# MatteoSoldini/metamorphic_testing_of_the_MUSICA_Algorithm_for_x_ray_image_processing

Hardware: AMD Instinct MI355X
Metric: megapixels/sec full MUSICA pipeline (higher is better)
Workload: dtype f32

## Files before the change

devtools/random_parity.py:

```python
import os
import sys

ROOT = os.path.dirname(os.path.dirname(os.path.abspath(__file__)))
sys.path.insert(0, ROOT)
sys.path.insert(0, os.path.join(ROOT, "tests"))
import numpy as np
from metamorphic_testing_of_the_musica_algorithm_for_x_ray_image_processing_amd import processing as mp
from metamorphic_testing_of_the_musica_algorithm_for_x_ray_image_processing_amd.phantom import phantom
from oracle import binding as ob
import test_gpu_parity as tp

cases = int(sys.argv[1]) if len(sys.argv) > 1 else 30
rng = np.random.default_rng(int(sys.argv[2]) if len(sys.argv) > 2 else 7)
ob.set_threads(min(16, os.cpu_count() or 1))
knobs = ["MUSICA_SDEV_IN_EXPAND", "MUSICA_PAIR_RB_SDEV", "MUSICA_SDEV_ONE_LAUNCH", "MUSICA_GRAPH", "MUSICA_AUTOTUNE", "MUSICA_TINY_TAIL"]
for case in range(cases):
    n = int(rng.choice([8 * int(rng.integers(8, 190)), int(rng.integers(64, 1500))]))
    lmax = int(np.ceil(np.log2(n)))
    levels = int(rng.integers(4, lmax + 1))
    batch = int(rng.choice([1, 1, 2, 3]))
    clahe = bool(rng.integers(0, 4) == 0) and n >= 64
    linear = bool(rng.integers(0, 2))
    env = {k: str(int(rng.integers(0, 2))) for k in knobs}
    env["MUSICA_STREAMS"] = str(int(rng.integers(1, 3)))
    for k, v in env.items():
        os.environ[k] = v
    flags = (mp.FLAG_CLAHE if clahe else 0) | (mp.FLAG_LINEAR if linear else 0)
    px = np.stack([phantom(n, 5000 + 10 * case + k) for k in range(batch)])
    p = mp.MusicaProcessing()
    assert p.init(n, levels=levels, batch=batch, flags=flags), mp.last_error()
# ... 9 lines not shown
```

include/musica.h:

```cpp
#ifndef MUSICA_H
#define MUSICA_H

#include <stddef.h>
#include <stdint.h>

#ifdef __cplusplus
extern "C" {
#endif

#define MUSICA_ABI_VERSION 3

#define MUSICA_MAX_LEVELS 16
#define MUSICA_MIN_LEVELS 4
#define MUSICA_NOISE_BINS 2048
#define MUSICA_GRAD_BINS 1024
#define MUSICA_MAX_POINTS 256
#define MUSICA_CNR_LEVEL 3
#define MUSICA_COARSER_LEVELS_START 3
#define MUSICA_OUT_MARGIN 10
#define MUSICA_CLAHE_TILES 4
#define MUSICA_CLAHE_BINS 256

typedef struct musica_hist_max_point {
    uint32_t maxValue;
// ... 100 lines not shown

musica_ctx* musica_create(const musica_params* params);
musica_ctx* musica_create_ex(const musica_params* params, const musica_tunables* tunables);
void musica_tunables_default(musica_tunables* out);
int musica_get_tunables(const musica_ctx* ctx, musica_tunables* out);

void musica_destroy(musica_ctx* ctx);

uint32_t musica_get_image_size(const musica_ctx* ctx);
uint32_t musica_get_levels(const musica_ctx* ctx);
uint32_t musica_get_batch(const musica_ctx* ctx);
int musica_fuses_gradation_histogram(const musica_ctx* ctx);
int musica_fuses_reduce_band(const musica_ctx* ctx);
int musica_fuses_sdev(const musica_ctx* ctx);
int musica_get_paired_levels(const musica_ctx* ctx);
uint32_t musica_get_level_size(const musica_ctx* ctx, uint32_t level);
int musica_get_dispatch(const musica_ctx* ctx, int* streams, int* graph);


int musica_execute(musica_ctx* ctx, const uint16_t* pixels);

int musica_execute_device(musica_ctx* ctx, const uint16_t* d_pixels);

int musica_upload(musica_ctx* ctx, const uint16_t* pixels);
const uint16_t* musica_input_device_ptr(musica_ctx* ctx);

int musica_sync(musica_ctx* ctx);


int musica_get_graded(musica_ctx* ctx, float* dst);
// ... 233 lines not shown
```

metamorphic_testing_of_the_musica_algorithm_for_x_ray_image_processing_amd/csrc/kernels_pyramid.hip:

```cpp
#include <stdlib.h>
#include <type_traits>
#include "kernels_common.h"
#include "sdev_parts.h"
#include "launchers.h"

#ifndef MUSICA_PYRAMID_SD_ONLY
#define MUSICA_PYRAMID_FULL 1
#endif

namespace musica {

struct LaneCfg {
    int c;
    bool active;
    bool left_mirror;
    bool last_active;
    bool lane0, lane63;
    uint32_t off;
    uint32_t off_l;
    uint32_t off_r;
    uint32_t coff;
    uint32_t coff_l;
    uint32_t coff_r;
};
// ... 324 lines not shown
}
template <class R>
__device__ __forceinline__ void band_pair(const CRow& a, const CRow& b, const CRow& c, const R& fe, const R& fo, const LaneCfg& g,
                                          const Buf& bb, uint32_t off_e, uint32_t off_o) {
    float lowE[8], lowO[8], be[8], bo[8];
    lowpass_pair(a, b, c, g, lowE, lowO);
#pragma unroll
    for (int j = 0; j < 8; j++) {
        be[j] = fe.v[j] - lowE[j];
        bo[j] = fo.v[j] - lowO[j];
    }
    store8_nt(bb, g.off + off_e, be);
    store8_nt(bb, g.off + off_o, bo);
}

__device__ __forceinline__ uint32_t le090_bits(const FRowQ& fe, const FRowQ& fo) {
    uint32_t m = 0u;
#pragma unroll
    for (int j = 0; j < 8; j++) {
        m |= fe.v[j] <= 0.90f ? 1u << j : 0u;
        m |= fo.v[j] <= 0.90f ? 1u << (8 + j) : 0u;
    }
    return m;
}

__device__ __forceinline__ void load_f(FRow& r, const Buf& b, uint32_t row_off, uint32_t off, uint32_t off_h) {
    load8(r.v, b, off + row_off);
    const float4 h = bload4(b, off_h + row_off);
    r.h[0] = h.x; r.h[1] = h.y; r.h[2] = h.z; r.h[3] = h.w;
}

template <bool U16>
__device__ __forceinline__ void reduce_band_block(const void* __restrict__ fine, float* __restrict__ down, float* __restrict__ band,
                                                  int S, int pitch, size_t plane, int Sc, int cpitch, size_t cplane,
                                                  int rows_per_wave, const uint32_t* __restrict__ minmax, int min_chain_exact,
                                                  uint16_t* __restrict__ le090, const Tile tile, const int img) {
    const int lane = threadIdx.x & 63;
    const int seg = __builtin_amdgcn_readfirstlane((int)(tile.segblock * kWavesPerBlock + (threadIdx.x >> 6)));
    const int k0 = seg * rows_per_wave;
    if (k0 >= Sc) return;
    const int k1 = min(k0 + rows_per_wave, Sc);
    NormK nk = make_norm(0.0f, 1.0f);
    if (U16) {
        float minv, maxv;
        chain_scalars(minmax, img, min_chain_exact, minv, maxv);
        nk = make_norm(minv, maxv);
    }
    const Buf ib = U16 ? make_buf(reinterpret_cast<const uint16_t*>(fine) + (size_t)img * S * S, (size_t)S * S * 2)
                       : make_buf(reinterpret_cast<const float*>(fine) + (size_t)img * plane, plane * 4);
    const Buf db = make_buf(down + (size_t)img * cplane, cplane * 4);
    const Buf bb = make_buf(band + (size_t)img * plane, plane * 4);
    const LaneCfg g = make_cfg(tile.strip, lane, S);
    const bool want_mask = U16 && le090 != nullptr;
    const Buf mb = want_mask ? make_buf(le090 + (size_t)img * Sc * (S / 8), (size_t)Sc * (S / 8) * 2) : bb;
    const uint32_t moff = g.off == kOob ? kOob : (uint32_t)g.c >> 2, mrb = (uint32_t)S >> 2;
    const uint32_t px_bytes = U16 ? 2u : 4u;
    const uint32_t foff = g.off == kOob ? kOob : (uint32_t)g.c * px_bytes;
    const uint32_t foff_h = g.off_l != kOob ? (uint32_t)(g.c - 4) * px_bytes : (g.off_r != kOob ? (uint32_t)(g.c + 8) * px_bytes : kOob);
    const uint32_t qi = (uint32_t)lane & 3u;
    const int hi = S - 1;
    const uint32_t frb = U16 ? (uint32_t)S * 2u : (uint32_t)pitch * 4u, rb = (uint32_t)pitch * 4u, crb = (uint32_t)cpitch * 4u;
    const int ks = max(k0 - 1, 0), ke = min(k1, Sc - 1);

    typename std::conditional<U16, FRowQ, FRow>::type w0, w1, w2, w3, w4;
    RawF ra, rc;
    if constexpr (U16) {
        load_raw_f(ra, ib, (uint32_t)mirror_idx(2 * ks - 2, hi) * frb, foff, foff_h);
        convert_f(w0, ra, nk, qi);
        load_raw_f(ra, ib, (uint32_t)mirror_idx(2 * ks - 1, hi) * frb, foff, foff_h);
        convert_f(w1, ra, nk, qi);
        load_raw_f(ra, ib, (uint32_t)(2 * ks) * frb, foff, foff_h);
        convert_f(w2, ra, nk, qi);
        load_raw_f(ra, ib, (uint32_t)mirror_idx(2 * ks + 1, hi) * frb, foff, foff_h);
        load_raw_f(rc, ib, (uint32_t)mirror_idx(2 * ks + 2, hi) * frb, foff, foff_h);
    } else {
        load_f(w0, ib, (uint32_t)mirror_idx(2 * ks - 2, hi) * frb, foff, foff_h);
        load_f(w1, ib, (uint32_t)mirror_idx(2 * ks - 1, hi) * frb, foff, foff_h);
        load_f(w2, ib, (uint32_t)(2 * ks) * frb, foff, foff_h);
    }
    CRow c0, cm1, cm2;
    cm1 = CRow(); cm2 = CRow();
    for (int k = ks; k <= ke; k++) {
        if constexpr (U16) {
            convert_f(w3, ra, nk, qi);
            convert_f(w4, rc, nk, qi);
            const int kn = min(k + 1, ke);
            load_raw_f(ra, ib, (uint32_t)mirror_idx(2 * kn + 1, hi) * frb, foff, foff_h);
            load_raw_f(rc, ib, (uint32_t)mirror_idx(2 * kn + 2, hi) * frb, foff, foff_h);
        } else {
            load_f(w3, ib, (uint32_t)mirror_idx(2 * k + 1, hi) * frb, foff, foff_h);
            load_f(w4, ib, (uint32_t)mirror_idx(2 * k + 2, hi) * frb, foff, foff_h);
        }
        coarse_row(c0, w0, w1, w2, w3, w4, g);
        if (k >= k0 && k < k1)
            bstore4_nt(db, g.coff + (uint32_t)k * crb, make_float4(c0.v[0], c0.v[1], c0.v[2], c0.v[3]));
        const int kp = k - 1;
        if (kp >= k0 && kp < k1) {
            if constexpr (U16) if (want_mask) bstore_u16(mb, moff + (uint32_t)kp * mrb, le090_bits(w0, w1));
            band_pair(kp == 0 ? c0 : cm2, cm1, c0, w0, w1, g, bb, (uint32_t)(2 * kp) * rb, (uint32_t)(2 * kp + 1) * rb);
        }
        cm2 = cm1; cm1 = c0;
        w0 = w2; w1 = w3; w2 = w4;
    }
    if (k1 == Sc) {
        if constexpr (U16) if (want_mask) bstore_u16(mb, moff + (uint32_t)(Sc - 1) * mrb, le090_bits(w0, w1));
        band_pair(cm2, cm1, cm1, w0, w1, g, bb, (uint32_t)(2 * (Sc - 1)) * rb, (uint32_t)(2 * (Sc - 1) + 1) * rb);
    }
}
template <bool U16>
__global__ __launch_bounds__(kBlockThreads, 4) void k_reduce_band(const void* __restrict__ fine, float* __restrict__ down, float* __restrict__ band,
                                                               int S, int pitch, size_t plane, int Sc, int cpitch, size_t cplane,
                                                               int rows_per_wave, const uint32_t* __restrict__ minmax, int min_chain_exact,
                                                               uint16_t* __restrict__ le090, int swz) {
    reduce_band_block<U16>(fine, down, band, S, pitch, plane, Sc, cpitch, cplane, rows_per_wave, minmax, min_chain_exact, le090, xcd_tile(swz), (int)blockIdx.z);
}

__device__ __forceinline__ float lowpass_generic(const float* __restrict__ coarse, int cpitch, int Sc, int S, int x, int y, int ref) {
    if (ref) {
        float pixel = 0.0f;
#pragma unroll
        for (int m = 0; m < 5; m++) {
// ... 526 lines not shown
    return dim3(strips, (segs + kWavesPerBlock - 1) / kWavesPerBlock, batch);
}

#ifndef MUSICA_PYRAMID_FULL
__device__ __forceinline__ bool role_tile(int local, int strips, int blocks, int swz, Tile& t) {
    if (swz && (blocks & 7) == 0) {
        const int xcd = local & 7, j = local >> 3;
        t.strip = j % strips;
        t.segblock = xcd * (blocks >> 3) + j / strips;
    } else {
        t.strip = local % strips;
        t.segblock = local / strips;
    }
    return t.segblock < blocks;
}
__global__ __launch_bounds__(kBlockThreads, 4) void k_rb_sdev(const RbSdevArgs a) {
    __shared__ uint32_t lh[kHistLdsWords];
    __shared__ unsigned long long nzw[kWavesPerBlock][8];
    const int img = (int)blockIdx.z;
    Tile tile;
    if ((int)blockIdx.x >= a.rb_first) {
        if (!role_tile((int)blockIdx.x - a.rb_first, a.rb_strips, a.rb_blocks, a.swz, tile)) return;
        reduce_band_block<false>(a.fine, a.down, a.band, a.S, a.pitch, a.plane, a.Sc, a.cpitch, a.cplane, a.rows_rb, nullptr, 0, nullptr, tile, img);
        return;
    }
    const SdevRunLevel& l = a.sl;
    if (!role_tile((int)blockIdx.x, l.strips, l.blocks, a.swz, tile)) return;
    float* sd = l.sdev ? l.sdev + (size_t)img * l.plane : nullptr;
    if (l.rows > 0) sdev_march_block<true, true>(l.band + (size_t)img * l.plane, sd, l.S, l.pitch, l.plane, l.hist + (size_t)img * a.hist_stride, a.cov, l.rows, tile, lh);
    else sdev_run_block<true>(l.band + (size_t)img * l.plane, sd, l.S, l.pitch, l.plane, l.hist + (size_t)img * a.hist_stride, a.cov, tile, lh, nzw);
}
void launch_rb_sdev(hipStream_t st, RbSdevArgs a, const LevelDesc& ls, int batch) {
    const int s_strips = (ls.S + kStripCols - 1) / kStripCols;
    int s_blocks;
    if (a.sl.rows > 0) { const int segs = (ls.S + a.sl.rows - 1) / a.sl.rows; s_blocks = (segs + kWavesPerBlock - 1) / kWavesPerBlock; }
    else s_blocks = (ls.S + kHistArea - 1) / kHistArea;
    a.sl.plane = ls.plane; a.sl.S = ls.S; a.sl.pitch = ls.pitch; a.sl.strips = s_strips; a.sl.blocks = s_blocks; a.sl.first = 0;
    a.rb_first = (s_strips * s_blocks + 7) & ~7;
    a.rb_strips = (a.S + kStripCols - 1) / kStripCols;
    const int segs = (a.Sc + a.rows_rb - 1) / a.rows_rb;
    a.rb_blocks = (segs + kWavesPerBlock - 1) / kWavesPerBlock;
    const int total = a.rb_first + ((a.rb_strips * a.rb_blocks + 7) & ~7);
    hipLaunchKernelGGL(k_rb_sdev, dim3(total, 1, batch), dim3(kBlockThreads), 0, st, a);
}

void launch_expand_sd(hipStream_t st, const ExpandArgs& a, bool nr, int batch) {
    const dim3 grid = stream_grid(a.S, a.Sc, a.rows_per_wave, batch);
    if (nr && a.ghist) {
        if (a.chist) hipLaunchKernelGGL((k_expand_fast<GAIN_CURVE, true, true, MUSICA_SD_CH_W, true, true>), grid, dim3(kBlockThreads), 0, st, a);
        else hipLaunchKernelGGL((k_expand_fast<GAIN_CURVE, true, true, MUSICA_SD_W, false, true>), grid, dim3(kBlockThreads), 0, st, a);
// ... 89 lines not shown
```

metamorphic_testing_of_the_musica_algorithm_for_x_ray_image_processing_amd/csrc/launchers.h:

```cpp
#pragma once

#include <stdlib.h>
#include "musica_device.h"

namespace musica {

enum { GAIN_CONST = 0, GAIN_RANGE = 1, GAIN_CURVE = 2 };

struct ExpandArgs {
    const float* prev;
    const float* band;
    const float* sdev;
    const float* cnr;
    float* recon;
    const DevCurve* curves;
    const DevCurveLut* luts;
    int S, pitch; size_t plane;
    int Sc, cpitch; size_t cplane;
    int cnrS, cnrPitch; size_t cnrPlane;
    int cnrScale;
    float high;
    float lowCnr, lowFactor, highCnr, highFactor;
    int rows_per_wave;
    size_t curve_stride;
// ... 25 lines not shown
void launch_reduce(hipStream_t st, const float* in, const LevelDesc& li, float* out, const LevelDesc& lo, int batch, bool force_generic, int tag,
                   int swz, int regions, int ref = 0);
void launch_band(hipStream_t st, const float* fine, const float* coarse, float* band, const LevelDesc& lf, const LevelDesc& lc, int batch, int ref = 0);
void launch_reduce_band_u16(hipStream_t st, const uint16_t* px, float* down, float* band, const LevelDesc& lf, const LevelDesc& lc, int batch,
                            int rows_per_wave, const uint32_t* minmax, int min_chain_exact, uint16_t* le090, int swz);
void launch_reduce_band(hipStream_t st, const float* fine, float* down, float* band, const LevelDesc& lf, const LevelDesc& lc, int batch, int rows_per_wave,
                        int swz);
void launch_lowpass(hipStream_t st, const float* coarse, float* low, const LevelDesc& lf, const LevelDesc& lc, int batch, int ref = 0);
void launch_expand(hipStream_t st, const ExpandArgs& a, int gain_mode, bool nr, int batch, bool force_generic);
struct RbSdevArgs {
    const float* fine; float* down; float* band;
    int S, pitch; size_t plane; int Sc, cpitch; size_t cplane; int rows_rb;
    int rb_strips, rb_blocks, rb_first;
    SdevRunLevel sl;
    size_t hist_stride; int cov, swz;
};
void launch_rb_sdev(hipStream_t st, RbSdevArgs a, const LevelDesc& ls, int batch);
void launch_expand_sd(hipStream_t st, const ExpandArgs& a, bool nr, int batch);
void launch_tiny_tail(hipStream_t st, const TailArgs& a, int batch);
void launch_exp_band(hipStream_t st, const ExpandArgs& a, int gain_mode, bool nr, int batch);
void launch_clear(hipStream_t st, uint32_t* minmax, uint32_t* noise_hist, uint32_t* grad_hist, uint32_t* clahe_hist, int batch, uint32_t* grad_hist_b = nullptr, uint32_t* gzero = nullptr);
constexpr int kMinMaxSlots = 4096;
void launch_minmax(hipStream_t st, const uint16_t* px, int N, uint32_t* minmax, uint32_t* slots, uint32_t* ticket, int batch,
                   uint32_t* noise_hist = nullptr, uint32_t* grad_hist = nullptr, uint32_t* grad_hist_b = nullptr, uint32_t* gzero = nullptr,
                   uint32_t* clahe_hist = nullptr);
void launch_normalize(hipStream_t st, const uint16_t* px, float* out, const LevelDesc& l0, const uint32_t* minmax, int min_chain_exact, int batch);
void launch_sqrt(hipStream_t st, const uint16_t* px, float* out, const LevelDesc& l0, int batch);
void launch_sdev_hist(hipStream_t st, const float* band, float* sdev, const LevelDesc& l, uint32_t* hist, size_t hist_stride, int cov, int batch, int rows_per_wave, int swz);
void launch_sdev_hist_runs(hipStream_t st, int n, const float* const* band, float* const* sdev, const LevelDesc* lv, uint32_t* const* hist,
                           size_t hist_stride, int cov, int batch);
void launch_sdev_hist_levels(hipStream_t st, int n, const float* const* band, float* const* sdev, const LevelDesc* lv, uint32_t* const* hist,
                             const int* rows, size_t hist_stride, int cov, int batch, int swz);
// ... 154 lines not shown
```

metamorphic_testing_of_the_musica_algorithm_for_x_ray_image_processing_amd/csrc/musica_ctx.h:

```cpp
#pragma once

#include <algorithm>
#include <exception>
#include <vector>

#include "launchers.h"

using namespace musica;

__attribute__((visibility("hidden"))) int fail(const char* fmt, ...);

#define ABI_TRY try {
#define ABI_CATCH(name_)                                                                             \
    }                                                                                                \
    catch (const std::exception& e_) { return fail("%s: %s", name_, e_.what()); }                   \
    catch (...) { return fail("%s: unknown C++ exception", name_); }

#define HIP_OK(call)                                                                       \
    do {                                                                                   \
        hipError_t e_ = (call);                                                            \
        if (e_ != hipSuccess) return fail("%s failed: %s", #call, hipGetErrorString(e_));  \
    } while (0)

struct ProfSpan {
// ... 107 lines not shown
    const uint16_t* graph_input[kGraphSlots] = {};
    uint64_t graph_used[kGraphSlots] = {};
    uint64_t graph_clock = 0;
    int dag;
    uint16_t* d_input2 = nullptr;
    hipStream_t copy_stream = nullptr;
    hipEvent_t ev_copied[2] = {}, ev_consumed[2] = {};
    const uint16_t* cur_input = nullptr;
    musica_contrast_params* d_cparams = nullptr;
    uint32_t* d_plot = nullptr;
    bool fuse_gh;
    bool sd_fused, sd_active = false, sdev_stored = true;
    bool pair_rb_sdev;
    bool sdev_one_launch;
    int rows_rb[MUSICA_MAX_LEVELS];
    int xcd_swizzle;
    int xcd_regions;
    uint8_t* d_out8 = nullptr;
    uint8_t* h_out8 = nullptr;
    uint8_t* h_bmp = nullptr;
    StudyState study;
    uint16_t* d_input_kept = nullptr;
    bool stepped = false;
    hipEvent_t ev_caller = nullptr, ev_signal = nullptr;
    musica_contrast_params h_cparams[MUSICA_MAX_LEVELS];
    musica_nr_params h_nr[3];
    int rows_expand[MUSICA_MAX_LEVELS], rows_sdev[4];
    int expand_rows, sdev_rows, grad_groups, min_waves;
    uint32_t profiling = 0;
    std::vector<ProfSpan> spans;
// ... 88 lines not shown
```

metamorphic_testing_of_the_musica_algorithm_for_x_ray_image_processing_amd/csrc/musica_ctx.hip:

```cpp
#include <math.h>
#include <stdarg.h>
#include <stdio.h>
#include <stdlib.h>
#include <string.h>

#include <chrono>
#include <string>

#include "musica_ctx.h"

extern "C" int musica_write_bmp_gray(const char* path, uint32_t w, uint32_t h, const uint8_t* data);
extern "C" uint32_t musica_bmp24_header(uint32_t w, uint32_t h, uint8_t hdr[54]);
extern "C" int musica_write_file(const char* path, const uint8_t* bytes, size_t count);

static thread_local std::string g_last_error;

int fail(const char* fmt, ...) {
    char buf[512];
    va_list ap;
    va_start(ap, fmt);
    vsnprintf(buf, sizeof(buf), fmt, ap);
    va_end(ap);
    g_last_error = buf;
    fprintf(stderr, "MUSICA ERROR: %s\n", buf);
// ... 39 lines not shown

static musica_nr_params host_nr_params(uint32_t i, const musica_tunables& t) {
    const float nrHighCnr = t.nr_high_cnr, nrMaxHighFactor = t.nr_max_high_factor, nrLowCnr = t.nr_low_cnr, nrMinLowFactor = t.nr_min_low_factor;
    musica_nr_params q;
    q.highCnr = nrHighCnr;
    q.highFactor = nrMaxHighFactor - (nrMaxHighFactor - 1.0f) * ((float)i / (float)MUSICA_CNR_LEVEL);
    q.lowCnr = nrLowCnr;
    q.lowFactor = nrMinLowFactor + (1.0f - nrMinLowFactor) * ((float)i / (float)MUSICA_CNR_LEVEL);
    return q;
}

static void autotune(musica_ctx* c);
static bool rb_level(const musica_ctx* c, int i);
static int tail_first(const musica_ctx* c);
static int rb_sdev_pairs(const musica_ctx* c, int T);
static void copy_rows(musica_ctx* dst, const musica_ctx* src) {
    if (dst == src) return;
    memcpy(dst->rows_expand, src->rows_expand, sizeof(src->rows_expand));
    memcpy(dst->rows_sdev, src->rows_sdev, sizeof(src->rows_sdev));
    memcpy(dst->rows_rb, src->rows_rb, sizeof(src->rows_rb));
}

static uint32_t cnr_scale(int S, int cnrS) { return (uint32_t)ceilf((float)S / (float)cnrS); }

static int g_min_waves = 2048;
static int pick_rows(int dflt, int min_rows, int S, int rows_total, int batch, int min_waves = 0) {
    int rpw = dflt;
    const int strips = (S + kStripCols - 1) / kStripCols;
    if (min_waves <= 0) min_waves = g_min_waves;
    while (rpw > min_rows) {
// ... 166 lines not shown
    c->fuse_u16 = (N % 8) == 0 && !c->generic;
    c->clahe_raw = (params->flags & MUSICA_FLAG_CLAHE) && c->fuse_u16 && (N % 4) == 0 && env_int("MUSICA_CLAHE_FUSE", 1) != 0 &&
                   (cnr_scale(c->lv[0].S, c->lv[MUSICA_CNR_LEVEL].S) % 4) == 0;
    c->clahe_in_expand = env_int("MUSICA_CLAHE_IN_EXPAND", 1) != 0;
    c->clahe_one_apply = env_int("MUSICA_CLAHE_ONE_APPLY", 1) != 0;
    c->tiny_tail = env_int("MUSICA_TINY_TAIL", 1) != 0;
    c->grad_one_launch = env_int("MUSICA_GRAD_ONE_LAUNCH", 1) != 0;
    c->xcd_swizzle = env_int("MUSICA_XCD_SWIZZLE", 1) != 0 ? 1 : 0;
    c->xcd_regions = env_int("MUSICA_XCD_REGIONS", 1) != 0 ? 1 : 0;
    {
        const size_t texels = (size_t)c->B * N * N;
        const bool pays = texels >= ((params->flags & MUSICA_FLAG_LINEAR) ? (size_t)2 : (size_t)8) * 2048 * 2048;
        c->sd_fused = env_int("MUSICA_SDEV_IN_EXPAND", pays ? 1 : 0) != 0 && !c->generic;
    }
    c->pair_rb_sdev = env_int("MUSICA_PAIR_RB_SDEV", ((params->flags & MUSICA_FLAG_LINEAR) && (size_t)c->B * N * N >= (size_t)2 * 2048 * 2048) ? 1 : 0) != 0;
    c->sdev_one_launch = env_int("MUSICA_SDEV_ONE_LAUNCH", ((params->flags & MUSICA_FLAG_LINEAR) || c->B > 1) ? 1 : 0) != 0;
    c->fuse_gh = env_int("MUSICA_FUSE_GH", 1) != 0 && c->fuse_u16 && (!(params->flags & MUSICA_FLAG_CLAHE) || c->clahe_raw) &&
                 cnr_scale(c->lv[0].S, c->lv[MUSICA_CNR_LEVEL].S) == 8;
    tick.lap("streams + events");
    for_each_buffer(*c, *c, [&](auto& ptr, size_t count) { if (count) ok = ok && dalloc(c, &ptr, B * count); });
    ok = ok && dalloc(c, &c->d_cparams, (size_t)L);
    ok = ok && dalloc(c, &c->d_plot, (size_t)MUSICA_HIST_RENDER_WIDTH * MUSICA_HIST_RENDER_HEIGHT);
    tick.lap("device buffers");
    ok = ok && hipMemcpy(c->d_cparams, c->h_cparams, sizeof(musica_contrast_params) * L, hipMemcpyHostToDevice) == hipSuccess;
    tick.lap("parameter upload");
    if (!ok) {
        fail("musica_create: device allocation failed (%s)", hipGetErrorString(hipGetLastError()));
        musica_destroy(c);
        return nullptr;
    }
// ... 5 lines not shown
    return c;
}

uint32_t musica_get_image_size(const musica_ctx* c) { return c ? (uint32_t)c->N : 0; }
uint32_t musica_get_levels(const musica_ctx* c) { return c ? (uint32_t)c->L : 0; }
uint32_t musica_get_batch(const musica_ctx* c) { return c ? (uint32_t)c->B : 0; }
int musica_get_dispatch(const musica_ctx* c, int* streams, int* graph) {
    if (!c) return 0;
    if (streams) *streams = c->dag == 0 ? 1 : 2;
    if (graph) *graph = c->use_graph ? 1 : 0;
    return 1;
}
int musica_fuses_gradation_histogram(const musica_ctx* c) { return (c && c->fuse_gh && !c->generic) ? 1 : 0; }
int musica_fuses_reduce_band(const musica_ctx* c) { return (c && rb_level(c, 0)) ? 1 : 0; }
int musica_fuses_sdev(const musica_ctx* c) { return (c && c->sd_fused && rb_level(c, 0)) ? 1 : 0; }
int musica_get_paired_levels(const musica_ctx* c) { return (c && c->dag == 0) ? rb_sdev_pairs(c, tail_first(c)) : 0; }
uint32_t musica_get_level_size(const musica_ctx* c, uint32_t level) { return (c && (int)level <= c->L) ? (uint32_t)c->lv[level].S : 0; }

}

struct Span {
    musica_ctx* c;
    ProfSpan* s;
    hipStream_t st;
    Span(musica_ctx* ctx, int id) : c(ctx), s(nullptr), st(ctx->cur) {
        if (!((c->profiling >> id) & 1u)) return;
        if (c->spans_used == c->spans.size()) {
            ProfSpan n;
            n.id = id;
            hipEventCreate(&n.a);
// ... 30 lines not shown
    }
    c->norm_valid = false;
    if (!c->fuse_u16 || (c->d_clahe_hist && !c->clahe_raw)) {
        Span sp(c, MUSICA_KERNEL_NORMALIZE);
        launch_normalize(c->stream, c->cur_input, c->d_norm, c->lv[0], c->d_minmax, c->min_chain_exact, c->B);
        c->norm_valid = true;
    }
}
static void ensure_normalized(musica_ctx* c) {
    if (c->norm_valid) return;
    launch_normalize(c->stream, c->cur_input, c->d_norm, c->lv[0], c->d_minmax, c->min_chain_exact, c->B);
    c->norm_valid = true;
}

static bool rb_level(const musica_ctx* c, int i) { return !c->generic && c->lv[i].S >= 8 && (c->lv[i].S % 8) == 0; }
static void run_reduce_band(musica_ctx* c, int i, int rows) {
    if (i == 0)
        launch_reduce_band_u16(c->cur, c->cur_input, c->d_down[0], c->d_band[0], c->lv[0], c->lv[1], c->B, rows, c->d_minmax, c->min_chain_exact, c->d_le090,
                               c->xcd_swizzle);
    else
        launch_reduce_band(c->cur, level_input(c, i), c->d_down[i], c->d_band[i], c->lv[i], c->lv[i + 1], c->B, rows, c->xcd_swizzle);
}
static void run_reduce_and_band(musica_ctx* c, int i) {
    if (rb_level(c, i)) { Span sp(c, i == 0 ? MUSICA_KERNEL_REDUCE_L0 : MUSICA_KERNEL_REDUCE_REST); run_reduce_band(c, i, c->rows_rb[i]); return; }
    { Span sp(c, i == 0 ? MUSICA_KERNEL_REDUCE_L0 : MUSICA_KERNEL_REDUCE_REST); launch_reduce(c->cur, level_input(c, i), c->lv[i], c->d_down[i], c->lv[i + 1], c->B, true, i == 0 ? 0 : 1, c->xcd_swizzle, c->xcd_regions, c->ref_order); }
    { Span sp(c, i == 0 ? MUSICA_KERNEL_BAND_L0 : MUSICA_KERNEL_BAND_REST); launch_band(c->cur, level_input(c, i), c->d_down[i], c->d_band[i], c->lv[i], c->lv[i + 1], c->B, c->ref_order); }
}
static bool sd_level(const musica_ctx* c, int i) { return c->sd_active && i < MUSICA_CNR_LEVEL && rb_level(c, i); }
static void run_sdev_level(musica_ctx* c, int i, int rows) {
    if (c->ref_order) {
        launch_sdev_literal(c->cur, c->d_band[i], c->d_sdev[i], c->lv[i], c->B);
        launch_noise_hist_only(c->cur, c->d_sdev[i], c->lv[i], c->d_noise_hist + (size_t)i * MUSICA_NOISE_BINS, (size_t)4 * MUSICA_NOISE_BINS, c->hist_cov, c->B);
// ... 63 lines not shown
    const float* band[kSdevRunLevelsMax];
    float* sdev[kSdevRunLevelsMax];
    uint32_t* hist[kSdevRunLevelsMax];
    LevelDesc lv[kSdevRunLevelsMax];
    int rows[kSdevRunLevelsMax];
    int n = 0;
    for (int i = first; i <= MUSICA_CNR_LEVEL; i++, n++) {
        band[n] = c->d_band[i]; sdev[n] = sd_level(c, i) ? nullptr : c->d_sdev[i]; lv[n] = c->lv[i];
        hist[n] = c->d_noise_hist + (size_t)i * MUSICA_NOISE_BINS;
        rows[n] = c->rows_sdev[i] > 0 ? c->rows_sdev[i] : 0;
    }
    launch_sdev_hist_levels(c->cur, n, band, sdev, lv, hist, rows, (size_t)4 * MUSICA_NOISE_BINS, c->hist_cov, c->B, c->xcd_swizzle);
}
static void enqueue_analysis(musica_ctx* c, hipStream_t st = nullptr) {
    if (!st) st = c->stream;
    if (c->sdev_one_launch && !c->ref_order && !c->tuning) {
        { Span sp(c, MUSICA_KERNEL_SDEV_HIST); run_sdev_all_levels(c); }
        Span sp2(c, MUSICA_KERNEL_CURVES);
        launch_curves_cnr(st, c->d_noise_hist, (size_t)4 * MUSICA_NOISE_BINS, c->d_noise_max, c->d_curves, c->d_cparams, c->L, c->B, c->d_luts,
                          c->d_sdev[MUSICA_CNR_LEVEL], c->d_cnr, c->lv[MUSICA_CNR_LEVEL], c->d_minmax, c->min_chain_exact, c->d_thr090);
        return;
    }
    int merged = sdev_runs_from(c);
    if (merged >= MUSICA_CNR_LEVEL) merged = MUSICA_CNR_LEVEL + 1;
    for (int i = 0; i < merged; i++) {
        Span sp(c, MUSICA_KERNEL_SDEV_HIST);
        run_sdev_level(c, i, c->rows_sdev[i]);
    }
    if (merged <= MUSICA_CNR_LEVEL) {
        Span sp(c, MUSICA_KERNEL_SDEV_HIST);
        run_sdev_levels(c, merged);
    }
    {
        Span sp(c, MUSICA_KERNEL_CURVES);
        launch_curves_cnr(st, c->d_noise_hist, (size_t)4 * MUSICA_NOISE_BINS, c->d_noise_max, c->d_curves, c->d_cparams, c->L, c->B, c->d_luts,
                          c->d_sdev[MUSICA_CNR_LEVEL], c->d_cnr, c->lv[MUSICA_CNR_LEVEL], c->d_minmax, c->min_chain_exact, c->d_thr090);
    }
}

static ExpandArgs expand_args(musica_ctx* c, int lvl, float* dst) {
// ... 89 lines not shown
        return;
    }
    { Span sp(c, MUSICA_KERNEL_GRAD_APPLY); launch_grad_apply(c->stream, c->d_recon[0], c->d_graded, l0, c->d_gcurve, c->B); }
}

static void run_rb_sdev_pair(musica_ctx* c, int i) {
    const int r = i + 1;
    RbSdevArgs a;
    a.fine = level_input(c, r); a.down = c->d_down[r]; a.band = c->d_band[r];
    a.S = c->lv[r].S; a.pitch = c->lv[r].pitch; a.plane = c->lv[r].plane;
    a.Sc = c->lv[r + 1].S; a.cpitch = c->lv[r + 1].pitch; a.cplane = c->lv[r + 1].plane;
    a.rows_rb = c->rows_rb[r];
    a.sl.band = c->d_band[i]; a.sl.sdev = sd_level(c, i) ? nullptr : c->d_sdev[i];
    a.sl.hist = c->d_noise_hist + (size_t)i * MUSICA_NOISE_BINS;
    a.sl.rows = c->rows_sdev[i] > 0 ? c->rows_sdev[i] : 0;
    a.hist_stride = (size_t)4 * MUSICA_NOISE_BINS; a.cov = c->hist_cov; a.swz = c->xcd_swizzle;
    launch_rb_sdev(c->cur, a, c->lv[i], c->B);
}
static bool pairs_rb_sdev(const musica_ctx* c) { return c->pair_rb_sdev && !c->ref_order && !c->generic && !c->tuning; }
static int rb_sdev_pairs(const musica_ctx* c, int T) {
    if (!pairs_rb_sdev(c)) return 0;
    int n = 0;
    while (n <= MUSICA_CNR_LEVEL && n + 1 < T && rb_level(c, n) && rb_level(c, n + 1)) n++;
    return n;
}
static void enqueue_linear_paired(musica_ctx* c) {
    c->cur = c->stream;
    enqueue_norm(c, true);
    const int T = tail_first(c);
    run_reduce_and_band(c, 0);
    const int pairs = rb_sdev_pairs(c, T);
    int i = 0;
    for (; i < pairs; i++) {
        Span sp(c, MUSICA_KERNEL_SDEV_HIST);
        run_rb_sdev_pair(c, i);
    }
    for (int r = i + 1; r < T; r++) run_reduce_and_band(c, r);
    if (T < c->L) run_tiny_tail(c, T);
    if (i <= MUSICA_CNR_LEVEL) { Span sp(c, MUSICA_KERNEL_SDEV_HIST); run_sdev_all_levels(c, i); }
    {
        Span sp(c, MUSICA_KERNEL_CURVES);
        launch_curves_cnr(c->stream, c->d_noise_hist, (size_t)4 * MUSICA_NOISE_BINS, c->d_noise_max, c->d_curves, c->d_cparams, c->L, c->B, c->d_luts,
                          c->d_sdev[MUSICA_CNR_LEVEL], c->d_cnr, c->lv[MUSICA_CNR_LEVEL], c->d_minmax, c->min_chain_exact, c->d_thr090);
    }
    enqueue_expand(c, true, T - 1);
    enqueue_gradation(c, true);
}
static void enqueue_linear(musica_ctx* c) {
    if (pairs_rb_sdev(c)) { enqueue_linear_paired(c); return; }
    c->cur = c->stream;
    enqueue_norm(c, true);
    const int T = enqueue_reduce_from(c, 0);
    enqueue_analysis(c);
// ... 1130 lines not shown
```

metamorphic_testing_of_the_musica_algorithm_for_x_ray_image_processing_amd/processing.py:

```python
import ctypes as C
import math
import os

import numpy as np

_HERE = os.path.dirname(os.path.abspath(__file__))
LIB_PATH = os.path.join(_HERE, "libmusica_hip.so")
CLI_PATH = os.path.join(_HERE, "musica-standalone")

MAX_POINTS = 256
NOISE_BINS = 2048
GRAD_BINS = 1024
OUT_MARGIN = 10

HIST_RENDER_WIDTH, HIST_RENDER_HEIGHT = 512, 128

FLAG_CLAHE = 0x1
FLAG_NO_GRAPH = 0x2
FLAG_GENERIC_KERNELS = 0x4
FLAG_NO_AUTOTUNE = 0x8
FLAG_LINEAR = 0x10
FLAG_REFERENCE_ORDER = 0x20
FLAG_ONE_SHOT = 0x40

# ... 221 lines not shown


_VP = C.c_void_p
_U8P, _U16P, _U32P, _F32P = C.POINTER(C.c_uint8), C.POINTER(C.c_uint16), C.POINTER(C.c_uint32), C.POINTER(C.c_float)
ABI = {
    "musica_create": (_VP, [C.POINTER(Params)]),
    "musica_destroy": (None, [_VP]),
    "musica_get_image_size": (C.c_uint32, [_VP]),
    "musica_get_levels": (C.c_uint32, [_VP]),
    "musica_get_batch": (C.c_uint32, [_VP]),
    "musica_get_level_size": (C.c_uint32, [_VP, C.c_uint32]),
    "musica_fuses_gradation_histogram": (C.c_int, [_VP]),
    "musica_fuses_reduce_band": (C.c_int, [_VP]),
    "musica_fuses_sdev": (C.c_int, [_VP]),
    "musica_get_paired_levels": (C.c_int, [_VP]),
    "musica_get_dispatch": (C.c_int, [_VP, C.POINTER(C.c_int), C.POINTER(C.c_int)]),
    "musica_execute": (C.c_int, [_VP, _U16P]),
    "musica_execute_device": (C.c_int, [_VP, _VP]),
    "musica_execute_stream": (C.c_int, [_VP, C.POINTER(_VP), C.c_uint32, C.POINTER(Stats)]),
    "musica_host_alloc": (_VP, [_VP, C.c_size_t]),
    "musica_host_free": (None, [_VP, _VP]),
    "musica_upload": (C.c_int, [_VP, _U16P]),
    "musica_input_device_ptr": (_VP, [_VP]),
    "musica_sync": (C.c_int, [_VP]),
    "musica_get_graded": (C.c_int, [_VP, _F32P]),
    "musica_save_out_image": (C.c_int, [_VP, C.c_uint32, C.c_char_p]),
    "musica_get_out_pixels": (C.c_int, [_VP, C.c_uint32, _U8P]),
    "musica_get_image": (C.c_int, [_VP, C.c_uint32, C.c_int, C.c_uint32, _F32P]),
    "musica_image_side": (C.c_uint32, [_VP, C.c_int, C.c_uint32]),
    "musica_get_noise_hist": (C.c_int, [_VP, C.c_uint32, C.c_uint32, _U32P]),
# ... 317 lines not shown
        self._ok(self._lib.musica_get_clahe_hist(self._h, image_index, out.ctypes.data_as(_U32P)), "musica_get_clahe_hist")
        return out

    def clahe_curves(self, image_index=0):
        out = np.empty((4, 4, 256, 2), dtype=np.float32)
        self._ok(self._lib.musica_get_clahe_curves(self._h, image_index, C.cast(out.ctypes.data, C.POINTER(Point))), "musica_get_clahe_curves")
        return out

    def dispatch(self):
        st, g = C.c_int(0), C.c_int(0)
        self._lib.musica_get_dispatch(self._h, C.byref(st), C.byref(g))
        return st.value, bool(g.value)

    def dispatch_text(self):
        st, g = self.dispatch()
        return "%s, %s" % ({1: "one stream", 2: "two streams (analysis beside the reduce tail)"}[st],
                           "hipGraph replay" if g else "eager launches")

    def fuses_gradhist(self):
        return self._lib.musica_fuses_gradation_histogram(self._h) == 1

    def fuses_sdev(self):
        return self._lib.musica_fuses_sdev(self._h) == 1

    def paired_levels(self):
        return self._lib.musica_get_paired_levels(self._h)

    def fuses_reduce_band(self):
        return self._lib.musica_fuses_reduce_band(self._h) == 1

    def export_out(self, d_dst, first=0, count=None, fmt=OUT_U8, row_pitch=0, image_pitch=0):
        count = self.batch - int(first) if count is None else int(count)
        rows, width = out_geometry(self.imageSize, fmt)
        row_pitch = int(row_pitch) or width
        image_pitch = int(image_pitch) or row_pitch * rows
        self._ok(self._lib.musica_export_out(self._h, int(first), count, int(fmt), d_dst, row_pitch, image_pitch), "musica_export_out")

    def stream_wait(self, stream=None):
# ... 414 lines not shown
```

Measured before the change: 120,600.

## Fuse level-0 noise histogram into the reduce+band kernel with seam fix-up pass

Adds a reduce+band kernel variant for level 0 that squares the band rows it already holds in registers and runs the local-sdev histogram scan in the same pass. Because strips cannot see their neighbours' columns, a separate seam kernel re-reads band values around strip boundaries to finish the histogram. The aim is to avoid a second full read of the level-0 band for the noise histogram. The cost is extra halo rows per wave, higher register pressure (launch bounds lowered to 2 waves), and an extra seam launch. It is enabled by default only when the picked row count is 16 and dag==0.

```diff
diff --git a/devtools/random_parity.py b/devtools/random_parity.py
--- a/devtools/random_parity.py
+++ b/devtools/random_parity.py
@@ -13,7 +13,7 @@
 cases = int(sys.argv[1]) if len(sys.argv) > 1 else 30
 rng = np.random.default_rng(int(sys.argv[2]) if len(sys.argv) > 2 else 7)
 ob.set_threads(min(16, os.cpu_count() or 1))
-knobs = ["MUSICA_SDEV_IN_EXPAND", "MUSICA_PAIR_RB_SDEV", "MUSICA_SDEV_ONE_LAUNCH", "MUSICA_GRAPH", "MUSICA_AUTOTUNE", "MUSICA_TINY_TAIL"]
+knobs = ["MUSICA_SDEV_IN_EXPAND", "MUSICA_HIST_IN_RB", "MUSICA_PAIR_RB_SDEV", "MUSICA_SDEV_ONE_LAUNCH", "MUSICA_GRAPH", "MUSICA_AUTOTUNE", "MUSICA_TINY_TAIL"]
 for case in range(cases):
     n = int(rng.choice([8 * int(rng.integers(8, 190)), int(rng.integers(64, 1500))]))
     lmax = int(np.ceil(np.log2(n)))
diff --git a/include/musica.h b/include/musica.h
--- a/include/musica.h
+++ b/include/musica.h
@@ -138,6 +138,7 @@
 int musica_fuses_reduce_band(const musica_ctx* ctx);
 int musica_fuses_sdev(const musica_ctx* ctx);
 int musica_get_paired_levels(const musica_ctx* ctx);
+int musica_fuses_noise_hist(const musica_ctx* ctx);
 uint32_t musica_get_level_size(const musica_ctx* ctx, uint32_t level);
 int musica_get_dispatch(const musica_ctx* ctx, int* streams, int* graph);
 
diff --git a/metamorphic_testing_of_the_musica_algorithm_for_x_ray_image_processing_amd/csrc/kernels_pyramid.hip b/metamorphic_testing_of_the_musica_algorithm_for_x_ray_image_processing_amd/csrc/kernels_pyramid.hip
--- a/metamorphic_testing_of_the_musica_algorithm_for_x_ray_image_processing_amd/csrc/kernels_pyramid.hip
+++ b/metamorphic_testing_of_the_musica_algorithm_for_x_ray_image_processing_amd/csrc/kernels_pyramid.hip
@@ -362,6 +362,29 @@
     store8_nt(bb, g.off + off_o, bo);
 }
 
+template <class R>
+__device__ __forceinline__ void band_pair_sq(const CRow& a, const CRow& b, const CRow& c, const R& fe, const R& fo, const LaneCfg& g,
+                                             const Buf& bb, uint32_t off_e, uint32_t off_o, bool store, SRow& se, SRow& so) {
+    float lowE[8], lowO[8], be[8], bo[8];
+    lowpass_pair(a, b, c, g, lowE, lowO);
+#pragma unroll
+    for (int j = 0; j < 8; j++) {
+        be[j] = fe.v[j] - lowE[j];
+        bo[j] = fo.v[j] - lowO[j];
+    }
+    if (store) {
+        store8_nt(bb, g.off + off_e, be);
+        store8_nt(bb, g.off + off_o, bo);
+    }
+#pragma unroll
+    for (int j = 0; j < 8; j++) {
+        const float te = g.active ? be[j] : 0.0f, to = g.active ? bo[j] : 0.0f;
+        se.q[j] = te * te;
+        so.q[j] = to * to;
+    }
+    se.e0 = se.e1 = so.e0 = so.e1 = 0.0f;
+}
+
 __device__ __forceinline__ uint32_t le090_bits(const FRowQ& fe, const FRowQ& fo) {
     uint32_t m = 0u;
 #pragma unroll
@@ -378,11 +401,13 @@
     r.h[0] = h.x; r.h[1] = h.y; r.h[2] = h.z; r.h[3] = h.w;
 }
 
-template <bool U16>
+template <bool U16, bool NH = false>
 __device__ __forceinline__ void reduce_band_block(const void* __restrict__ fine, float* __restrict__ down, float* __restrict__ band,
                                                   int S, int pitch, size_t plane, int Sc, int cpitch, size_t cplane,
                                                   int rows_per_wave, const uint32_t* __restrict__ minmax, int min_chain_exact,
-                                                  uint16_t* __restrict__ le090, const Tile tile, const int img) {
+                                                  uint16_t* __restrict__ le090, const Tile tile, const int img,
+                                                  uint32_t* lh = nullptr, int cov = 0) {
+    static_assert(!NH || U16, "the histogram form is level 0's");
     const int lane = threadIdx.x & 63;
     const int seg = __builtin_amdgcn_readfirstlane((int)(tile.segblock * kWavesPerBlock + (threadIdx.x >> 6)));
     const int k0 = seg * rows_per_wave;
@@ -408,7 +433,7 @@
     const uint32_t qi = (uint32_t)lane & 3u;
     const int hi = S - 1;
     const uint32_t frb = U16 ? (uint32_t)S * 2u : (uint32_t)pitch * 4u, rb = (uint32_t)pitch * 4u, crb = (uint32_t)cpitch * 4u;
-    const int ks = max(k0 - 1, 0), ke = min(k1, Sc - 1);
+    const int ks = max(k0 - (NH ? 2 : 1), 0), ke = min(k1 + (NH ? 1 : 0), Sc - 1);
 
     typename std::conditional<U16, FRowQ, FRow>::type w0, w1, w2, w3, w4;
     RawF ra, rc;
@@ -428,6 +453,21 @@
     }
     CRow c0, cm1, cm2;
     cm1 = CRow(); cm2 = CRow();
+    [[maybe_unused]] SRow q0 = SRow(), q1 = SRow(), q2 = SRow(), q3 = SRow(), q4 = SRow(), q5 = SRow();
+    [[maybe_unused]] unsigned long long alive[8], start[8];
+    [[maybe_unused]] const SCfg sg = make_scfg(tile.strip, lane, S);
+    if constexpr (NH) {
+        sdev_start_masks(start, alive, sg, cov);
+        const unsigned long long keep_l = tile.strip > 0 ? ~1ull : ~0ull, keep_r = (tile.strip + 1) * kStripCols < S ? ~(1ull << 63) : ~0ull;
+        start[0] &= keep_l; start[1] &= keep_l; start[6] &= keep_r; start[7] &= keep_r;
+    }
+    [[maybe_unused]] auto scan_pair = [&](int kq) {
+        if (kq >= k0 && kq < k1) {
+            sdev_row<true, true>(q0, q1, q2, q3, q4, sg, S, 2 * kq, cov, nullptr, bb, 0u, lh, alive, start, false);
+            sdev_row<true, true>(q1, q2, q3, q4, q5, sg, S, 2 * kq + 1, cov, nullptr, bb, 0u, lh, alive, start, false);
+        }
+        q0 = q2; q1 = q3; q2 = q4; q3 = q5;
+    };
     for (int k = ks; k <= ke; k++) {
         if constexpr (U16) {
             convert_f(w3, ra, nk, qi);
@@ -443,7 +483,14 @@
         if (k >= k0 && k < k1)
             bstore4_nt(db, g.coff + (uint32_t)k * crb, make_float4(c0.v[0], c0.v[1], c0.v[2], c0.v[3]));
         const int kp = k - 1;
-        if (kp >= k0 && kp < k1) {
+        if constexpr (NH) {
+            if (kp >= max(k0 - 1, 0)) {
+                const bool mine = kp >= k0 && kp < k1;
+                if (want_mask && mine) bstore_u16(mb, moff + (uint32_t)kp * mrb, le090_bits(w0, w1));
+                band_pair_sq(kp == 0 ? c0 : cm2, cm1, c0, w0, w1, g, bb, (uint32_t)(2 * kp) * rb, (uint32_t)(2 * kp + 1) * rb, mine, q4, q5);
+                scan_pair(kp - 1);
+            }
+        } else if (kp >= k0 && kp < k1) {
             if constexpr (U16) if (want_mask) bstore_u16(mb, moff + (uint32_t)kp * mrb, le090_bits(w0, w1));
             band_pair(kp == 0 ? c0 : cm2, cm1, c0, w0, w1, g, bb, (uint32_t)(2 * kp) * rb, (uint32_t)(2 * kp + 1) * rb);
         }
@@ -452,7 +499,14 @@
     }
     if (k1 == Sc) {
         if constexpr (U16) if (want_mask) bstore_u16(mb, moff + (uint32_t)(Sc - 1) * mrb, le090_bits(w0, w1));
-        band_pair(cm2, cm1, cm1, w0, w1, g, bb, (uint32_t)(2 * (Sc - 1)) * rb, (uint32_t)(2 * (Sc - 1) + 1) * rb);
+        if constexpr (NH) {
+            band_pair_sq(cm2, cm1, cm1, w0, w1, g, bb, (uint32_t)(2 * (Sc - 1)) * rb, (uint32_t)(2 * (Sc - 1) + 1) * rb, true, q4, q5);
+            scan_pair(Sc - 2);
+            q4 = SRow(); q5 = SRow();
+            scan_pair(Sc - 1);
+        } else {
+            band_pair(cm2, cm1, cm1, w0, w1, g, bb, (uint32_t)(2 * (Sc - 1)) * rb, (uint32_t)(2 * (Sc - 1) + 1) * rb);
+        }
     }
 }
 template <bool U16>
@@ -1009,6 +1063,82 @@
     }
     return t.segblock < blocks;
 }
+__device__ __forceinline__ void hist_seam_block(const float* __restrict__ band, int S, int pitch, uint32_t* __restrict__ hist, int cov,
+                                                int first, int items, uint32_t* lh) {
+    hist_lds_clear(lh);
+    __syncthreads();
+    const int w = first + (int)threadIdx.x;
+    const int bounds = (S + kStripCols - 1) / kStripCols - 1;
+    const int ci = w & 3, b = (w >> 2) % bounds + 1, run = (w >> 2) / bounds;
+    const int x = b * kStripCols - 2 + ci, y0 = run * kHistArea;
+    if (w < items && x < cov && y0 < cov) {
+        float q[kHistArea + 4][5];
+#pragma unroll
+        for (int r = 0; r < kHistArea + 4; r++) {
+            const int y = y0 - 2 + r;
+            const bool in = y >= 0 && y < S;
+            const float* row = band + (size_t)(in ? y : 0) * pitch + (x - 2);
+#pragma unroll
+            for (int m = 0; m < 5; m++) {
+                const float v = in ? row[m] : 0.0f;
+                q[r][m] = v * v;
+            }
+        }
+        const uint32_t copy = (uint32_t)((threadIdx.x % kHistCopies) * kHistCopyStride);
+        bool alive = true;
+#pragma unroll
+        for (int r = 0; r < kHistArea; r++) {
+            float c[5];
+#pragma unroll
+            for (int m = 0; m < 5; m++) c[m] = sum5(q[r][m], q[r + 1][m], q[r + 2][m], q[r + 3][m], q[r + 4][m]);
+            const float s = sqrtf(sum5(c[0], c[1], c[2], c[3], c[4]) / 25.0f);
+            const int bin = musica_noise_bin(s);
+            alive = alive && bin != 0 && y0 + r < S;
+            if (alive) atomicAdd(&lh[copy + (uint32_t)bin], 1u);
+        }
+    }
+    __syncthreads();
+    hist_lds_flush(lh, hist);
+}
+__global__ __launch_bounds__(kBlockThreads) void k_hist_seam(const float* __restrict__ band, int S, int pitch, size_t plane, uint32_t* __restrict__ hist,
+                                                             size_t hist_stride, int cov, int items) {
+    __shared__ uint32_t lh[kHistLdsWords];
+    const int img = (int)blockIdx.z;
+    hist_seam_block(band + (size_t)img * plane, S, pitch, hist + (size_t)img * hist_stride, cov, (int)blockIdx.x * kBlockThreads, items, lh);
+}
+static inline int seam_items(int S, int cov) {
+    const int bounds = (S + kStripCols - 1) / kStripCols - 1, rows = S < cov ? S : cov;
+    return 4 * bounds * ((rows + kHistArea - 1) / kHistArea);
+}
+void launch_hist_seam(hipStream_t st, const float* band, const LevelDesc& l, uint32_t* hist, size_t hist_stride, int cov, int batch) {
+    const int items = seam_items(l.S, cov);
+    if (items <= 0) return;
+    hipLaunchKernelGGL(k_hist_seam, dim3((items + kBlockThreads - 1) / kBlockThreads, 1, batch), dim3(kBlockThreads), 0, st, band, l.S, l.pitch, l.plane,
+                       hist, hist_stride, cov, items);
+}
+
+#ifndef MUSICA_RB_HIST_W
+#define MUSICA_RB_HIST_W 2
+#endif
+__global__ __launch_bounds__(kBlockThreads, MUSICA_RB_HIST_W) void k_reduce_band_hist(const void* __restrict__ fine, float* __restrict__ down, float* __restrict__ band,
+                                                               int S, int pitch, size_t plane, int Sc, int cpitch, size_t cplane,
+                                                               int rows_per_wave, const uint32_t* __restrict__ minmax, int min_chain_exact,
+                                                               uint16_t* __restrict__ le090, int swz, uint32_t* __restrict__ hist, size_t hist_stride, int cov) {
+    __shared__ uint32_t lh[kHistLdsWords];
+    hist_lds_clear(lh);
+    __syncthreads();
+    reduce_band_block<true, true>(fine, down, band, S, pitch, plane, Sc, cpitch, cplane, rows_per_wave, minmax, min_chain_exact, le090, xcd_tile(swz),
+                                  (int)blockIdx.z, lh, cov);
+    __syncthreads();
+    hist_lds_flush(lh, hist + (size_t)blockIdx.z * hist_stride);
+}
+void launch_reduce_band_u16_hist(hipStream_t st, const uint16_t* px, float* down, float* band, const LevelDesc& lf, const LevelDesc& lc, int batch,
+                                 int rows_per_wave, const uint32_t* minmax, int min_chain_exact, uint16_t* le090, int swz, uint32_t* hist,
+                                 size_t hist_stride, int cov) {
+    hipLaunchKernelGGL(k_reduce_band_hist, stream_grid(lf.S, lc.S, rows_per_wave, batch), dim3(kBlockThreads), 0, st, (const void*)px, down, band, lf.S,
+                       lf.pitch, lf.plane, lc.S, lc.pitch, lc.plane, rows_per_wave, minmax, min_chain_exact, le090, swz, hist, hist_stride, cov);
+}
+
 __global__ __launch_bounds__(kBlockThreads, 4) void k_rb_sdev(const RbSdevArgs a) {
     __shared__ uint32_t lh[kHistLdsWords];
     __shared__ unsigned long long nzw[kWavesPerBlock][8];
@@ -1020,15 +1150,22 @@
         return;
     }
     const SdevRunLevel& l = a.sl;
+    if (l.rows < 0) {
+        if ((int)blockIdx.x < l.blocks)
+            hist_seam_block(l.band + (size_t)img * l.plane, l.S, l.pitch, l.hist + (size_t)img * a.hist_stride, a.cov, (int)blockIdx.x * kBlockThreads, a.seam_items, lh);
+        return;
+    }
     if (!role_tile((int)blockIdx.x, l.strips, l.blocks, a.swz, tile)) return;
     float* sd = l.sdev ? l.sdev + (size_t)img * l.plane : nullptr;
     if (l.rows > 0) sdev_march_block<true, true>(l.band + (size_t)img * l.plane, sd, l.S, l.pitch, l.plane, l.hist + (size_t)img * a.hist_stride, a.cov, l.rows, tile, lh);
     else sdev_run_block<true>(l.band + (size_t)img * l.plane, sd, l.S, l.pitch, l.plane, l.hist + (size_t)img * a.hist_stride, a.cov, tile, lh, nzw);
 }
 void launch_rb_sdev(hipStream_t st, RbSdevArgs a, const LevelDesc& ls, int batch) {
-    const int s_strips = (ls.S + kStripCols - 1) / kStripCols;
+    int s_strips = (ls.S + kStripCols - 1) / kStripCols;
     int s_blocks;
-    if (a.sl.rows > 0) { const int segs = (ls.S + a.sl.rows - 1) / a.sl.rows; s_blocks = (segs + kWavesPerBlock - 1) / kWavesPerBlock; }
+    a.seam_items = 0;
+    if (a.sl.rows < 0) { a.seam_items = seam_items(ls.S, a.cov); s_strips = 1; s_blocks = (a.seam_items + kBlockThreads - 1) / kBlockThreads; }
+    else if (a.sl.rows > 0) { const int segs = (ls.S + a.sl.rows - 1) / a.sl.rows; s_blocks = (segs + kWavesPerBlock - 1) / kWavesPerBlock; }
     else s_blocks = (ls.S + kHistArea - 1) / kHistArea;
     a.sl.plane = ls.plane; a.sl.S = ls.S; a.sl.pitch = ls.pitch; a.sl.strips = s_strips; a.sl.blocks = s_blocks; a.sl.first = 0;
     a.rb_first = (s_strips * s_blocks + 7) & ~7;
diff --git a/metamorphic_testing_of_the_musica_algorithm_for_x_ray_image_processing_amd/csrc/launchers.h b/metamorphic_testing_of_the_musica_algorithm_for_x_ray_image_processing_amd/csrc/launchers.h
--- a/metamorphic_testing_of_the_musica_algorithm_for_x_ray_image_processing_amd/csrc/launchers.h
+++ b/metamorphic_testing_of_the_musica_algorithm_for_x_ray_image_processing_amd/csrc/launchers.h
@@ -63,8 +63,13 @@
     int rb_strips, rb_blocks, rb_first;
     SdevRunLevel sl;
     size_t hist_stride; int cov, swz;
+    int seam_items;
 };
 void launch_rb_sdev(hipStream_t st, RbSdevArgs a, const LevelDesc& ls, int batch);
+void launch_reduce_band_u16_hist(hipStream_t st, const uint16_t* px, float* down, float* band, const LevelDesc& lf, const LevelDesc& lc, int batch,
+                                 int rows_per_wave, const uint32_t* minmax, int min_chain_exact, uint16_t* le090, int swz, uint32_t* hist,
+                                 size_t hist_stride, int cov);
+void launch_hist_seam(hipStream_t st, const float* band, const LevelDesc& l, uint32_t* hist, size_t hist_stride, int cov, int batch);
 void launch_expand_sd(hipStream_t st, const ExpandArgs& a, bool nr, int batch);
 void launch_tiny_tail(hipStream_t st, const TailArgs& a, int batch);
 void launch_exp_band(hipStream_t st, const ExpandArgs& a, int gain_mode, bool nr, int batch);
diff --git a/metamorphic_testing_of_the_musica_algorithm_for_x_ray_image_processing_amd/csrc/musica_ctx.h b/metamorphic_testing_of_the_musica_algorithm_for_x_ray_image_processing_amd/csrc/musica_ctx.h
--- a/metamorphic_testing_of_the_musica_algorithm_for_x_ray_image_processing_amd/csrc/musica_ctx.h
+++ b/metamorphic_testing_of_the_musica_algorithm_for_x_ray_image_processing_amd/csrc/musica_ctx.h
@@ -145,6 +145,8 @@
     bool pair_rb_sdev;
     bool sdev_one_launch;
     int rows_rb[MUSICA_MAX_LEVELS];
+    int hist_in_rb;
+    int hist_rb_rows;
     int xcd_swizzle;
     int xcd_regions;
     uint8_t* d_out8 = nullptr;
diff --git a/metamorphic_testing_of_the_musica_algorithm_for_x_ray_image_processing_amd/csrc/musica_ctx.hip b/metamorphic_testing_of_the_musica_algorithm_for_x_ray_image_processing_amd/csrc/musica_ctx.hip
--- a/metamorphic_testing_of_the_musica_algorithm_for_x_ray_image_processing_amd/csrc/musica_ctx.hip
+++ b/metamorphic_testing_of_the_musica_algorithm_for_x_ray_image_processing_amd/csrc/musica_ctx.hip
@@ -77,6 +77,7 @@
 static bool rb_level(const musica_ctx* c, int i);
 static int tail_first(const musica_ctx* c);
 static int rb_sdev_pairs(const musica_ctx* c, int T);
+static int hist_rb_rows(const musica_ctx* c);
 static void copy_rows(musica_ctx* dst, const musica_ctx* src) {
     if (dst == src) return;
     memcpy(dst->rows_expand, src->rows_expand, sizeof(src->rows_expand));
@@ -273,6 +274,8 @@
         c->sd_fused = env_int("MUSICA_SDEV_IN_EXPAND", pays ? 1 : 0) != 0 && !c->generic;
     }
     c->pair_rb_sdev = env_int("MUSICA_PAIR_RB_SDEV", ((params->flags & MUSICA_FLAG_LINEAR) && (size_t)c->B * N * N >= (size_t)2 * 2048 * 2048) ? 1 : 0) != 0;
+    c->hist_in_rb = env_int("MUSICA_HIST_IN_RB", -1);
+    c->hist_rb_rows = env_int("MUSICA_HIST_RB_ROWS", 0) & ~7;
     c->sdev_one_launch = env_int("MUSICA_SDEV_ONE_LAUNCH", ((params->flags & MUSICA_FLAG_LINEAR) || c->B > 1) ? 1 : 0) != 0;
     c->fuse_gh = env_int("MUSICA_FUSE_GH", 1) != 0 && c->fuse_u16 && (!(params->flags & MUSICA_FLAG_CLAHE) || c->clahe_raw) &&
                  cnr_scale(c->lv[0].S, c->lv[MUSICA_CNR_LEVEL].S) == 8;
@@ -308,6 +311,9 @@
 int musica_fuses_gradation_histogram(const musica_ctx* c) { return (c && c->fuse_gh && !c->generic) ? 1 : 0; }
 int musica_fuses_reduce_band(const musica_ctx* c) { return (c && rb_level(c, 0)) ? 1 : 0; }
 int musica_fuses_sdev(const musica_ctx* c) { return (c && c->sd_fused && rb_level(c, 0)) ? 1 : 0; }
+int musica_fuses_noise_hist(const musica_ctx* c) {
+    return (c && c->sd_fused && !c->ref_order && !c->generic && c->fuse_u16 && rb_level(c, 0) && hist_rb_rows(c) > 0) ? 1 : 0;
+}
 int musica_get_paired_levels(const musica_ctx* c) { return (c && c->dag == 0) ? rb_sdev_pairs(c, tail_first(c)) : 0; }
 uint32_t musica_get_level_size(const musica_ctx* c, uint32_t level) { return (c && (int)level <= c->L) ? (uint32_t)c->lv[level].S : 0; }
 
@@ -368,8 +374,24 @@
 }
 
 static bool rb_level(const musica_ctx* c, int i) { return !c->generic && c->lv[i].S >= 8 && (c->lv[i].S % 8) == 0; }
+static int hist_rb_rows(const musica_ctx* c) {
+    if (c->hist_in_rb == 0 || c->hist_cov <= 0) return 0;
+    const int r = pick_rows(16, 8, c->lv[0].S, c->lv[1].S, c->B, 1024);
+    if (c->hist_in_rb < 0 && !(r == 16 && c->dag == 0)) return 0;
+    return c->hist_rb_rows > 0 ? c->hist_rb_rows : r;
+}
+static bool hist_in_rb(const musica_ctx* c) {
+    return c->sd_active && !c->tuning && !c->ref_order && !c->generic && c->fuse_u16 && rb_level(c, 0) && hist_rb_rows(c) > 0;
+}
+static uint32_t* noise_hist_of(const musica_ctx* c, int i) { return c->d_noise_hist + (size_t)i * MUSICA_NOISE_BINS; }
+static void run_hist_seam(musica_ctx* c) {
+    launch_hist_seam(c->cur, c->d_band[0], c->lv[0], noise_hist_of(c, 0), (size_t)4 * MUSICA_NOISE_BINS, c->hist_cov, c->B);
+}
 static void run_reduce_band(musica_ctx* c, int i, int rows) {
-    if (i == 0)
+    if (i == 0 && hist_in_rb(c))
+        launch_reduce_band_u16_hist(c->cur, c->cur_input, c->d_down[0], c->d_band[0], c->lv[0], c->lv[1], c->B, hist_rb_rows(c), c->d_minmax, c->min_chain_exact,
+                                    c->d_le090, c->xcd_swizzle, noise_hist_of(c, 0), (size_t)4 * MUSICA_NOISE_BINS, c->hist_cov);
+    else if (i == 0)
         launch_reduce_band_u16(c->cur, c->cur_input, c->d_down[0], c->d_band[0], c->lv[0], c->lv[1], c->B, rows, c->d_minmax, c->min_chain_exact, c->d_le090,
                                c->xcd_swizzle);
     else
@@ -463,16 +485,19 @@
 }
 static void enqueue_analysis(musica_ctx* c, hipStream_t st = nullptr) {
     if (!st) st = c->stream;
+    const int s0 = hist_in_rb(c) ? 1 : 0;
+    if (s0) { Span sp(c, MUSICA_KERNEL_SDEV_HIST); run_hist_seam(c); }
     if (c->sdev_one_launch && !c->ref_order && !c->tuning) {
-        { Span sp(c, MUSICA_KERNEL_SDEV_HIST); run_sdev_all_levels(c); }
+        { Span sp(c, MUSICA_KERNEL_SDEV_HIST); run_sdev_all_levels(c, s0); }
         Span sp2(c, MUSICA_KERNEL_CURVES);
         launch_curves_cnr(st, c->d_noise_hist, (size_t)4 * MUSICA_NOISE_BINS, c->d_noise_max, c->d_curves, c->d_cparams, c->L, c->B, c->d_luts,
                           c->d_sdev[MUSICA_CNR_LEVEL], c->d_cnr, c->lv[MUSICA_CNR_LEVEL], c->d_minmax, c->min_chain_exact, c->d_thr090);
         return;
     }
     int merged = sdev_runs_from(c);
+    if (merged < s0) merged = s0;
     if (merged >= MUSICA_CNR_LEVEL) merged = MUSICA_CNR_LEVEL + 1;
-    for (int i = 0; i < merged; i++) {
+    for (int i = s0; i < merged; i++) {
         Span sp(c, MUSICA_KERNEL_SDEV_HIST);
         run_sdev_level(c, i, c->rows_sdev[i]);
     }
@@ -592,6 +617,7 @@
     a.sl.band = c->d_band[i]; a.sl.sdev = sd_level(c, i) ? nullptr : c->d_sdev[i];
     a.sl.hist = c->d_noise_hist + (size_t)i * MUSICA_NOISE_BINS;
     a.sl.rows = c->rows_sdev[i] > 0 ? c->rows_sdev[i] : 0;
+    if (i == 0 && hist_in_rb(c)) a.sl.rows = -1;
     a.hist_stride = (size_t)4 * MUSICA_NOISE_BINS; a.cov = c->hist_cov; a.swz = c->xcd_swizzle;
     launch_rb_sdev(c->cur, a, c->lv[i], c->B);
 }
@@ -615,6 +641,7 @@
     }
     for (int r = i + 1; r < T; r++) run_reduce_and_band(c, r);
     if (T < c->L) run_tiny_tail(c, T);
+    if (i == 0 && hist_in_rb(c)) { Span sp(c, MUSICA_KERNEL_SDEV_HIST); run_hist_seam(c); i = 1; }
     if (i <= MUSICA_CNR_LEVEL) { Span sp(c, MUSICA_KERNEL_SDEV_HIST); run_sdev_all_levels(c, i); }
     {
         Span sp(c, MUSICA_KERNEL_CURVES);
diff --git a/metamorphic_testing_of_the_musica_algorithm_for_x_ray_image_processing_amd/processing.py b/metamorphic_testing_of_the_musica_algorithm_for_x_ray_image_processing_amd/processing.py
--- a/metamorphic_testing_of_the_musica_algorithm_for_x_ray_image_processing_amd/processing.py
+++ b/metamorphic_testing_of_the_musica_algorithm_for_x_ray_image_processing_amd/processing.py
@@ -259,6 +259,7 @@
     "musica_fuses_reduce_band": (C.c_int, [_VP]),
     "musica_fuses_sdev": (C.c_int, [_VP]),
     "musica_get_paired_levels": (C.c_int, [_VP]),
+    "musica_fuses_noise_hist": (C.c_int, [_VP]),
     "musica_get_dispatch": (C.c_int, [_VP, C.POINTER(C.c_int), C.POINTER(C.c_int)]),
     "musica_execute": (C.c_int, [_VP, _U16P]),
     "musica_execute_device": (C.c_int, [_VP, _VP]),
@@ -606,14 +607,20 @@
 
     def dispatch_text(self):
         st, g = self.dispatch()
-        return "%s, %s" % ({1: "one stream", 2: "two streams (analysis beside the reduce tail)"}[st],
-                           "hipGraph replay" if g else "eager launches")
+        text = "%s, %s" % ({1: "one stream", 2: "two streams (analysis beside the reduce tail)"}[st],
+                             "hipGraph replay" if g else "eager launches")
+        if self.fuses_noise_hist():
+            text += ", level-0 noise histogram inside reduce + band"
+        return text
 
     def fuses_gradhist(self):
         return self._lib.musica_fuses_gradation_histogram(self._h) == 1
 
     def fuses_sdev(self):
         return self._lib.musica_fuses_sdev(self._h) == 1
+
+    def fuses_noise_hist(self):
+        return self._lib.musica_fuses_noise_hist(self._h) == 1
 
     def paired_levels(self):
         return self._lib.musica_get_paired_levels(self._h)
```

Measured after the change: 124,400, median of 6. 1.03x the previous value.
